# JerryX1110/Robust-Video-Object-Segmentation

Measured on AMD Instinct MI355X. Metric: frames/sec, AOC-Net matching + calibration hot path (480p, 3 objects), higher is better.
Workload: dtype f32; 1 GPU; cfg2: 121x213 stride-4 maps (480p), O=4 (3 objects + background), K=16 proxies, C=100, 60-frame clips, MEM_EVERY=5 (pool R=1..12), 20 Lloyd iterations, local windows 2..12, 10 IA gates + 4 conditioning blocks; sequences_per_gpu=2, proxy_mode=reference

## Files before the change

### robust-video-object-segmentation_amd/csrc/labels_kmeans.hip

```cpp
#include "aoc_common.h"
#include <stdlib.h>
#include <algorithm>
#include <string.h>

namespace {

constexpr int LP_BLOCK = 256;

__global__ __launch_bounds__(LP_BLOCK) void label_flags_kernel(const float *__restrict__ labels, int n, int n_obj,
                                                                uint32_t *__restrict__ right_bits,
                                                                uint32_t *__restrict__ wrong_bits,
                                                                int32_t *__restrict__ block_counts, int n_blocks) {
    __shared__ int32_t wave_cnt[LP_BLOCK / 64][AOC_MAX_OBJECTS + 1];
    const int row = blockIdx.x * LP_BLOCK + threadIdx.x;
    uint32_t right = 0, wrong = 0;
    if (row < n) {
        const float *l = labels + (size_t)row * n_obj;
        float sum = 0.0f;
        for (int o = 0; o < n_obj; ++o) {
            float v = l[o];
            sum += v;
            if (v > 0.9f) right |= 1u << o;
            if (v < 0.1f) wrong |= 1u << o;
        }
// ... 2058 lines not shown
        if constexpr (NF > 1) { if (!skip[1]) { st[1] = ks_chunk_exact<1, NF>(to_float(1), cur, blocks_here, lane, ks_big); to_int(1); } }
        if constexpr (NF > 2) {
            if (!skip[2]) { st[2] = ks_chunk_exact<2, NF>(to_float(2), cur, blocks_here, lane, ks_big); to_int(2); }
            if (!skip[3]) { st[3] = ks_chunk_exact<3, NF>(to_float(3), cur, blocks_here, lane, ks_big); to_int(3); }
        }
        ks_tex += KS_CLK() - ks_tb;
        if (ks_big) KS_STAT(2, 1);
#pragma unroll
        for (int f = 0; f < NF; ++f) note_crossing(f, c, e_in[f]);
    }
#pragma unroll
    for (int f = 0; f < NF; ++f) st[f] = to_float(f);
    if (ks_big) { KS_STAT(0, KS_CLK() - ks_t0); KS_STAT(1, ks_tsum); KS_STAT(4, ks_tex); }
    if (lane == 0) {
        const float fc = (float)cnt;
#pragma unroll
        for (int f = 0; f < NF; ++f) out[f] = st[f] / fc;
        if (pred.e0) {
#pragma unroll
            for (int f = 0; f < NF; ++f) {
                const size_t idx = ((size_t)s * kmax + j) * C + NF * q + f;
                pred.e0[idx] = (int8_t)pe0[f];
#pragma unroll
                for (int i = 0; i < KP_CROSS; ++i) {
                    pred.cidx[idx * KP_CROSS + i] = (uint16_t)pci[f][i];
                    pred.ce[idx * KP_CROSS + i] = (int8_t)pce[f][i];
                }
            }
        }
    }
}

constexpr int OS_BATCH = 128;
constexpr int OS_FP = 7;
constexpr int OS_LD = 32;
constexpr int OS_NPROD = 7;
constexpr int OS_PP = OS_BATCH * OS_FP / (OS_NPROD * 64);
constexpr int OS_DEPTH = 6;
static_assert(OS_PP * OS_NPROD * 64 == OS_BATCH * OS_FP && OS_DEPTH % 2 == 0 && OS_FP * 4 <= OS_LD, "ordered-sum geometry");
inline int os_groups(int C) { return (C / 4 + OS_FP - 1) / OS_FP; }
__device__ __forceinline__ int os_groups_dev(int C) { return (C / 4 + OS_FP - 1) / OS_FP; }

template <int MODE>
__device__ __forceinline__ void os_ordered_sum_body(int j, int s, int grp, float *__restrict__ os_lds, const float *__restrict__ pool, uint32_t pool_bytes, int C,
                                                    const int32_t *__restrict__ seg_off, const int32_t *__restrict__ seg_k,
                                                    const int32_t *__restrict__ counts, const int32_t *__restrict__ cbase,
                                                    const uint32_t *__restrict__ moff, int kmax, float *__restrict__ dst,
                                                    int member_cap, float *__restrict__ head_state) {
    if (j >= seg_k[s]) return;
    const int oc = s * kmax + j;
    const int cnt_all = counts[oc];
    const int f0 = grp * OS_FP * 4;
    const int nfeat = min(OS_FP * 4, C - f0);
    float *out = ((MODE == 0) ? dst + (size_t)oc * C : dst + (((size_t)s * 2 + 1) * kmax + j) * C) + f0;
    if (cnt_all == 0) {
        if (MODE == 1 && (int)threadIdx.x < nfeat) out[threadIdx.x] = 0.0f;
        return;
    }
    const bool head_only = member_cap > 0 && cnt_all > member_cap;
    const int cnt = head_only ? member_cap : cnt_all;
    const int wave = threadIdx.x >> 6, lane = aoc_lane();
    const int nb = (cnt + OS_BATCH - 1) / OS_BATCH;

    if (wave == 0) {
        const bool active = lane < nfeat;
        const float *col = os_lds + (active ? lane : 0);
        float sum = 0.0f;
        for (int b = 0; b < nb; ++b) {
            __syncthreads();
            const float *t = col + (b & 1) * OS_BATCH * OS_LD;
            float xa[16], xb[16];
#pragma unroll
            for (int u = 0; u < 16; ++u) xa[u] = t[u * OS_LD];
#pragma unroll
            for (int g = 0; g < OS_BATCH / 16; g += 2) {
#pragma unroll
                for (int u = 0; u < 16; ++u) xb[u] = t[((g + 1) * 16 + u) * OS_LD];
#pragma unroll
                for (int u = 0; u < 16; ++u) sum = sum + xa[u];
                if (g + 2 < OS_BATCH / 16) {
#pragma unroll
                    for (int u = 0; u < 16; ++u) xa[u] = t[((g + 2) * 16 + u) * OS_LD];
                }
#pragma unroll
                for (int u = 0; u < 16; ++u) sum = sum + xb[u];
            }
        }
        if (active) {
            if (head_only) head_state[(size_t)oc * C + f0 + lane] = sum;
            else out[lane] = sum / (float)cnt;
        }
        return;
    }

    const uint32_t *list = moff + seg_off[s] + cbase[oc];
    __amdgpu_buffer_rsrc_t rsrc = __builtin_amdgcn_make_buffer_rsrc(const_cast<float *>(pool), 0, pool_bytes, 0x00020000);
    const int p = (wave - 1) * 64 + lane;
    const int c4 = C >> 2;
    int prow[OS_PP];
    uint32_t pbyte[OS_PP];
    bool pvalid[OS_PP];
#pragma unroll
    for (int i = 0; i < OS_PP; ++i) {
        const int idx = i * (OS_NPROD * 64) + p;
        prow[i] = idx / OS_FP;
        const int piece = idx - prow[i] * OS_FP;
        pvalid[i] = grp * OS_FP + piece < c4;
        pbyte[i] = (uint32_t)(grp * OS_FP + piece) * 16u;
    }
    auto load_offs = [&](int b, uint32_t (&o)[OS_PP]) {
#pragma unroll
        for (int i = 0; i < OS_PP; ++i) {
            const int m = b * OS_BATCH + prow[i];
            const uint32_t v = list[min(m, cnt - 1)];
            o[i] = (b < nb && pvalid[i] && m < cnt) ? v + pbyte[i] : KU_INVALID_OFF;
        }
    };
    auto load_rows = [&](const uint32_t (&o)[OS_PP], u32x4 (&d)[OS_PP]) {
#pragma unroll
        for (int i = 0; i < OS_PP; ++i) d[i] = __builtin_amdgcn_raw_buffer_load_b128(rsrc, o[i], 0, 0);
    };
    auto write_rows = [&](int b, const u32x4 (&d)[OS_PP]) {
        float *base = os_lds + (b & 1) * OS_BATCH * OS_LD;
#pragma unroll
        for (int i = 0; i < OS_PP; ++i)
            *reinterpret_cast<u32x4 *>(base + prow[i] * OS_LD + ((pbyte[i] >> 2) - f0)) = d[i];
    };
    u32x4 d[OS_DEPTH][OS_PP];
    uint32_t o[2][OS_PP];
    {
        uint32_t po[OS_DEPTH + 2][OS_PP];
#pragma unroll
        for (int k = 0; k < OS_DEPTH + 2; ++k) load_offs(k, po[k]);
#pragma unroll
        for (int k = 0; k < OS_DEPTH; ++k) load_rows(po[k], d[k]);
        write_rows(0, d[0]);
        load_rows(po[OS_DEPTH], d[0]);
#pragma unroll
        for (int i = 0; i < OS_PP; ++i) o[1][i] = po[OS_DEPTH + 1][i];
    }
    for (int b0 = 0; b0 < nb; b0 += OS_DEPTH) {
#pragma unroll
        for (int k = 0; k < OS_DEPTH; ++k) {
            const int b = b0 + k;
            if (b < nb) {
                __syncthreads();
                if (b + 1 < nb) write_rows(b + 1, d[(k + 1) % OS_DEPTH]);
                load_offs(b + 2 + OS_DEPTH, o[k & 1]);
                load_rows(o[(k + 1) & 1], d[(k + 1) % OS_DEPTH]);
            }
        }
    }
}
#ifndef AOC_OD_NPROD
#define AOC_OD_NPROD 3
#endif
#ifndef AOC_OD_DEPTH
#define AOC_OD_DEPTH 1
#endif
constexpr int OD_NPROD = AOC_OD_NPROD;
constexpr int OD_HALF = 64;
constexpr int OD_BATCH = OD_NPROD * OD_HALF;
constexpr int OD_DEPTH = AOC_OD_DEPTH;
constexpr int OD_NB = OD_DEPTH + 1;
constexpr int OD_LD = OS_FP * 4;
constexpr int OD_BATCH_BYTES = OD_BATCH * OD_LD * 4;
constexpr int OD_RING_FLOATS = OD_NB * OD_BATCH * OD_LD;
constexpr int OD_OPS = OS_FP + 1;
constexpr int OD_LDS_FLOATS = OD_RING_FLOATS + OD_NB * OD_BATCH;
static_assert(OD_DEPTH * OD_OPS < 64 && OD_NPROD >= 1 && OD_NPROD <= 3, "vmcnt is a 6-bit counter; the launch has four waves");

__device__ __forceinline__ void od_glds4(const void *gsrc, uint32_t lds_dst) {
    unsigned keep;
    asm volatile("s_mov_b32 %0, m0\n\ts_mov_b32 m0, %2\n\ts_nop 0\n\tglobal_load_lds_dword %1, off\n\ts_mov_b32 m0, %0"
                 : "=&s"(keep) : "v"(gsrc), "s"(lds_dst) : "memory");
}
__device__ __forceinline__ void od_glds16(uint32_t byte_off, const void *base, uint32_t lds_dst) {
    unsigned keep;
    asm volatile("s_mov_b32 %0, m0\n\ts_mov_b32 m0, %3\n\ts_nop 0\n\tglobal_load_lds_dwordx4 %1, %2\n\ts_mov_b32 m0, %0"
                 : "=&s"(keep) : "v"(byte_off), "s"(base), "s"(lds_dst) : "memory");
}
template <int N>
__device__ __forceinline__ void od_wait_vm() { asm volatile("s_waitcnt vmcnt(%0)" ::"n"(N) : "memory"); }
__device__ __forceinline__ void od_barrier() {
    __builtin_amdgcn_s_waitcnt(0xc07f);
    __builtin_amdgcn_s_barrier();
    asm volatile("" ::: "memory");
}

template <int MODE>
__device__ __forceinline__ void os_head_dma_body(int j, int s, int grp, float *__restrict__ os_lds, const float *__restrict__ pool, int C,
                                                 const int32_t *__restrict__ seg_off, const int32_t *__restrict__ seg_k,
                                                 const int32_t *__restrict__ counts, const int32_t *__restrict__ cbase,
                                                 const uint32_t *__restrict__ moff, int kmax, float *__restrict__ dst, int member_cap,
                                                 float *__restrict__ head_state, KsPred pred) {
    const int wave = __builtin_amdgcn_readfirstlane(threadIdx.x >> 6), lane = aoc_lane();
    if (wave > OD_NPROD) return;
    if (j >= seg_k[s]) return;
    const int oc = s * kmax + j;
    const int cnt_all = counts[oc];
    const int f0 = grp * OS_FP * 4;
    const int nfeat = min(OS_FP * 4, C - f0);
    float *out = ((MODE == 0) ? dst + (size_t)oc * C : dst + (((size_t)s * 2 + 1) * kmax + j) * C) + f0;
    if (cnt_all == 0) {
        if (MODE == 1 && (int)threadIdx.x < nfeat) out[threadIdx.x] = 0.0f;
        return;
    }
    const bool head_only = member_cap > 0 && cnt_all > member_cap;
    const int cnt = head_only ? member_cap : cnt_all;
    const int nb = (cnt + OD_BATCH - 1) / OD_BATCH;
    auto wrap = [](int x) { return x >= OD_NB ? x - OD_NB : x; };

    if (wave == 0) {
        const bool active = lane < nfeat;
        const float *col = os_lds + (active ? lane : 0);
        float sum = 0.0f;
        int slot = 0;
        for (int b = 0; b < nb; ++b) {
            od_barrier();
            const float *t = col + slot * (OD_BATCH * OD_LD);
            constexpr int OD_G = 32, NG = OD_BATCH / OD_G;
            const int rem = (b + 1 < nb) ? OD_BATCH : cnt - b * OD_BATCH;
            float xa[OD_G], xb[OD_G];
#pragma unroll
            for (int u = 0; u < OD_G; ++u) xa[u] = t[u * OD_LD];
#pragma unroll
            for (int g = 0; g < NG; g += 2) {
                if (g + 1 < NG) {
#pragma unroll
                    for (int u = 0; u < OD_G; ++u) xb[u] = t[((g + 1) * OD_G + u) * OD_LD];
                }
                if (rem >= (g + 1) * OD_G) {
#pragma unroll
                    for (int u = 0; u < OD_G; ++u) sum = sum + xa[u];
                } else {
#pragma unroll
                    for (int u = 0; u < OD_G; ++u) sum = sum + (g * OD_G + u < rem ? xa[u] : 0.0f);
                }
                if (g + 2 < NG) {
#pragma unroll
                    for (int u = 0; u < OD_G; ++u) xa[u] = t[((g + 2) * OD_G + u) * OD_LD];
                }
                if (g + 1 < NG) {
                    if (rem >= (g + 2) * OD_G) {
#pragma unroll
                        for (int u = 0; u < OD_G; ++u) sum = sum + xb[u];
                    } else {
#pragma unroll
                        for (int u = 0; u < OD_G; ++u) sum = sum + ((g + 1) * OD_G + u < rem ? xb[u] : 0.0f);
                    }
                }
            }
            slot = wrap(slot + 1);
        }
        if (active) {
            if (head_only) head_state[(size_t)oc * C + f0 + lane] = sum;
            else out[lane] = sum / (float)cnt;
            if (!head_only && pred.e0) {
                const size_t idx = (size_t)oc * C + f0 + lane;
                const KsBinade bb = ks_binade(sum);
                pred.e0[idx] = (int8_t)(bb.ok ? (int)((__float_as_uint(sum) >> 23) & 0xff) - 127 : KC_UNSAFE);
                pred.cidx[idx * KP_CROSS] = (uint16_t)0xFFFF;
            }
        }
        return;
    }

    const int p = wave - 1;
    const uint32_t *list = moff + seg_off[s] + cbase[oc];
    const uint32_t lds_base = (uint32_t)reinterpret_cast<uintptr_t>(os_lds);
    const uint32_t offs_base = lds_base + OD_RING_FLOATS * 4 + (uint32_t)p * (OD_HALF * 4);
    const uint32_t *offs = reinterpret_cast<const uint32_t *>(os_lds + OD_RING_FLOATS) + p * OD_HALF;
    const int npiece = min(OS_FP, (C >> 2) - grp * OS_FP);
    int prow[OS_FP];
    uint32_t pbyte[OS_FP];
#pragma unroll
    for (int i = 0; i < OS_FP; ++i) {
        const int idx = i * 64 + lane;
        prow[i] = idx / OS_FP;
        const int piece = idx - prow[i] * OS_FP;
        pbyte[i] = (uint32_t)(grp * OS_FP + (piece < npiece ? piece : 0)) * 16u;
    }
    auto issue_offs = [&](int b, int slot) {
        od_glds4(list + min(b * OD_BATCH + p * OD_HALF + lane, cnt - 1), offs_base + (uint32_t)slot * (OD_BATCH * 4));
    };
    auto issue_rows = [&](int slot) {
        const uint32_t *o = offs + slot * OD_BATCH;
        uint32_t src[OS_FP];
#pragma unroll
        for (int i = 0; i < OS_FP; ++i) src[i] = o[prow[i]] + pbyte[i];
        const uint32_t d = lds_base + (uint32_t)slot * OD_BATCH_BYTES + (uint32_t)p * (OD_HALF * OD_LD * 4);
#pragma unroll
        for (int i = 0; i < OS_FP; ++i) od_glds16(src[i], pool, d + (uint32_t)i * 1024u);
    };
#pragma unroll
    for (int x = 0; x < OD_DEPTH; ++x) issue_offs(x, x);
    od_wait_vm<0>();
#pragma unroll
    for (int i = 0; i < OD_DEPTH; ++i) {
        issue_offs(OD_DEPTH + i, wrap(OD_DEPTH + i));
        issue_rows(i);
    }
    int slot = 0;
    for (int b = 0; b < nb; ++b) {
        od_wait_vm<(OD_DEPTH - 1) * OD_OPS>();
        od_barrier();
        const int slot_d = wrap(slot + OD_DEPTH);
        issue_offs(b + 2 * OD_DEPTH, wrap(slot_d + OD_DEPTH));
        issue_rows(slot_d);
        slot = wrap(slot + 1);
    }
    od_wait_vm<0>();
}
template <int MODE>
__global__ __launch_bounds__((OS_NPROD + 1) * 64) void km_ordered_sum_kernel(const float *__restrict__ pool, uint32_t pool_bytes, int C,
                                                                              const int32_t *__restrict__ seg_off, const int32_t *__restrict__ seg_k,
                                                                              const int32_t *__restrict__ counts, const int32_t *__restrict__ cbase,
                                                                              const uint32_t *__restrict__ moff, int kmax, float *__restrict__ dst,
                                                                              int member_cap, float *__restrict__ head_state) {
    __shared__ __attribute__((aligned(16))) float os_lds[2 * OS_BATCH * OS_LD];
    os_ordered_sum_body<MODE>(blockIdx.x, blockIdx.y, blockIdx.z, os_lds, pool, pool_bytes, C, seg_off, seg_k, counts, cbase, moff, kmax, dst, member_cap, head_state);
}
template <int MODE, bool DMA>
__global__ __launch_bounds__(DMA ? 256 : (OS_NPROD + 1) * 64) void km_heads_chunk_sums_kernel(const float *__restrict__ pool, uint32_t pool_bytes, int C,
                                                                                   const int32_t *__restrict__ seg_off, const int32_t *__restrict__ seg_k,
                                                                                   const int32_t *__restrict__ counts, const int32_t *__restrict__ cbase,
                                                                                   const uint32_t *__restrict__ moff, int kmax, int n_seg, float *__restrict__ dst,
                                                                                   int member_cap, float *__restrict__ head_state,
                                                                                   const int32_t *__restrict__ owner_cluster, const int32_t *__restrict__ owner_local,
                                                                                   float *__restrict__ csum, int start_chunk, int xcd_aware,
                                                                                   KsPred pred, int spec_fold, int8_t *__restrict__ cexp,
                                                                                   int32_t *__restrict__ cinc0, int32_t *__restrict__ cinc1,
                                                                                   const int32_t *__restrict__ cchunk, int n_chunks_grid, int n_fold_groups) {
    __shared__ __attribute__((aligned(16))) float os_lds[DMA ? (OD_LDS_FLOATS > 2 * OS_BATCH * OS_LD ? OD_LDS_FLOATS : 2 * OS_BATCH * OS_LD) : 2 * OS_BATCH * OS_LD];
    static_assert(sizeof(float) * 2 * OS_BATCH * OS_LD >= sizeof(uint32_t) * KS_CHUNK + sizeof(float4) * 256, "the chunk role's buffers fit the head role's");
    static_assert(2 * OS_BATCH * OS_LD >= KC_FOLD_LDS_FLOATS, "the fold role's buffers fit the head role's");
    const int n_head = kmax * n_seg * os_groups_dev(C);
    const int b = blockIdx.x;
    if (b < n_head) {
        const int n_cl = kmax * n_seg, groups = os_groups_dev(C);
        const int blk = b / (8 * groups), rem = b - blk * (8 * groups);
        const int pc = min(8, n_cl - blk * 8);
        int grp = rem / pc, c = blk * 8 + rem - grp * pc;
        if (!xcd_aware) { c = b % n_cl; grp = b / n_cl; }
        const int j = c % kmax, s = c / kmax;
        if (DMA) os_head_dma_body<MODE>(j, s, grp, os_lds, pool, C, seg_off, seg_k, counts, cbase, moff, kmax, dst, member_cap, head_state, pred);
        else os_ordered_sum_body<MODE>(j, s, grp, os_lds, pool, pool_bytes, C, seg_off, seg_k, counts, cbase, moff, kmax, dst, member_cap, head_state);
        return;
    }
    if (threadIdx.x >= 256) return;
    if (DMA && spec_fold) {
        static_assert(!DMA || OD_LDS_FLOATS >= KC_WIDE_LDS_FLOATS, "the wide fold's tile fits the heads' ring");
        kc_chunk_fold_wide_body(b - n_head, os_lds, pool, C, seg_off, counts, cbase, moff, kmax, owner_cluster, owner_local, cexp, cinc0, cinc1, start_chunk,
                                n_chunks_grid, n_fold_groups, xcd_aware, pred);
        return;
    }
    uint32_t *loffs = reinterpret_cast<uint32_t *>(os_lds);
    float4 *part = reinterpret_cast<float4 *>(os_lds + KS_CHUNK);
    kc_chunk_sum_body(b - n_head, loffs, part, pool, C, seg_off, counts, cbase, moff, kmax, owner_cluster, owner_local, csum, start_chunk);
}

__global__ __launch_bounds__(64) void km_proxy_finish_kernel(const float *__restrict__ centroids, const int32_t *__restrict__ seg_k,
                                                              const int32_t *__restrict__ counts, int kmax, int C,
                                                              float *__restrict__ proxies, float *__restrict__ proxy_sqnorm) {
    const int s = blockIdx.y, j = blockIdx.x, lane = threadIdx.x;
    const int k = seg_k[s];
    float *p0 = proxies + (((size_t)s * 2 + 0) * kmax + j) * C;
    float *p1 = proxies + (((size_t)s * 2 + 1) * kmax + j) * C;
    if (j >= k) {
        for (int t = lane; t < C; t += 64) { p0[t] = 0.0f; p1[t] = 0.0f; }
        if (lane == 0) {
            proxy_sqnorm[((size_t)s * 2 + 0) * kmax + j] = INFINITY;
            proxy_sqnorm[((size_t)s * 2 + 1) * kmax + j] = INFINITY;
        }
        return;
    }
    const float *c = centroids + ((size_t)s * kmax + j) * C;
    float n0 = 0.0f, n1 = 0.0f;
    for (int t = lane; t < C; t += 64) {
        const float cv = c[t];
        p0[t] = cv;
        n0 += cv * cv;
        const float av = p1[t];
        n1 += av * av;
    }
    n0 = aoc_wave_sum(n0);
    n1 = aoc_wave_sum(n1);
    if (lane == 0) {
        proxy_sqnorm[((size_t)s * 2 + 0) * kmax + j] = n0;
        proxy_sqnorm[((size_t)s * 2 + 1) * kmax + j] = (counts[s * kmax + j] > 0) ? n1 : INFINITY;
    }
}

struct KsWorkspace {
    float *rownorm;
    uint16_t *rank16;
    int32_t *hist, *counts, *cbase;
    uint32_t *moff;
    int nb_max;
    int nch_cap;
    int32_t *cchunk, *owner_cluster, *owner_local, *cinc0, *cinc1;
    float *csum, *head;
    int8_t *cexp;
    uint32_t *cflag;
    int seg_chunks_max;
    KsPred pred;
};
inline size_t ks_pred_bytes(int n_seg, int kmax) {
    const size_t n = (size_t)n_seg * kmax * (AOC_MAX_CHANNELS / 2);
    return aoc_align_up(n, 256) + aoc_align_up(n * KP_CROSS * 2, 256) + aoc_align_up(n * KP_CROSS, 256);
}
inline int ks_chunk_capacity(int64_t cap, int n_seg, int kmax) { return (int)(cap / KS_CHUNK) + n_seg * (kmax + 1) + 2; }
inline size_t ks_workspace_bytes(int64_t cap, int n_seg, int kmax) {
    const size_t nb = (size_t)(cap + 255) / 256 + 1;
    const size_t nch = (size_t)ks_chunk_capacity(cap, n_seg, kmax);
    return aoc_align_up((size_t)cap * 4, 256) + aoc_align_up((size_t)cap * 2, 256) + aoc_align_up((size_t)n_seg * nb * kmax * 4, 256) +
           3 * aoc_align_up((size_t)n_seg * kmax * 4, 256) + aoc_align_up(((size_t)cap + 64) * 4, 256) + 2 * aoc_align_up(nch * 4, 256) +
           3 * aoc_align_up(nch * AOC_MAX_CHANNELS / 2 * 4, 256) + aoc_align_up(nch * AOC_MAX_CHANNELS / 2, 256) +
           aoc_align_up((size_t)n_seg * kmax * (AOC_MAX_CHANNELS / 2) * 4, 256) + aoc_align_up(nch * 8 * 4, 256) + ks_pred_bytes(n_seg, kmax);
}
inline KsWorkspace ks_carve(void *workspace, int64_t cap, int n_seg, int kmax, int64_t seg_bound = 0) {
    KsWorkspace w;
    char *p = static_cast<char *>(workspace);
    const size_t nb = (size_t)(cap + 255) / 256 + 1;
    w.nb_max = (int)((seg_bound > 0 && seg_bound < cap) ? (size_t)(seg_bound + 255) / 256 + 1 : nb);
    w.seg_chunks_max = (int)(((seg_bound > 0 && seg_bound < cap) ? seg_bound : cap) / KS_CHUNK + 1);
    w.rownorm = reinterpret_cast<float *>(p); p += aoc_align_up((size_t)cap * 4, 256);
    w.rank16 = reinterpret_cast<uint16_t *>(p); p += aoc_align_up((size_t)cap * 2, 256);
    w.hist = reinterpret_cast<int32_t *>(p); p += aoc_align_up((size_t)n_seg * nb * kmax * 4, 256);
    w.counts = reinterpret_cast<int32_t *>(p); p += aoc_align_up((size_t)n_seg * kmax * 4, 256);
    w.cbase = reinterpret_cast<int32_t *>(p); p += aoc_align_up((size_t)n_seg * kmax * 4, 256);
    w.cchunk = reinterpret_cast<int32_t *>(p); p += aoc_align_up((size_t)n_seg * kmax * 4, 256);
    w.moff = reinterpret_cast<uint32_t *>(p); p += aoc_align_up(((size_t)cap + 64) * 4, 256);
    const size_t nch = (size_t)ks_chunk_capacity(cap, n_seg, kmax);
    w.nch_cap = (int)nch;
    w.owner_cluster = reinterpret_cast<int32_t *>(p); p += aoc_align_up(nch * 4, 256);
    w.owner_local = reinterpret_cast<int32_t *>(p); p += aoc_align_up(nch * 4, 256);
    w.csum = reinterpret_cast<float *>(p); p += aoc_align_up(nch * AOC_MAX_CHANNELS / 2 * 4, 256);
    w.cinc0 = reinterpret_cast<int32_t *>(p); p += aoc_align_up(nch * AOC_MAX_CHANNELS / 2 * 4, 256);
    w.cinc1 = reinterpret_cast<int32_t *>(p); p += aoc_align_up(nch * AOC_MAX_CHANNELS / 2 * 4, 256);
    w.cexp = reinterpret_cast<int8_t *>(p); p += aoc_align_up(nch * AOC_MAX_CHANNELS / 2, 256);
    w.head = reinterpret_cast<float *>(p); p += aoc_align_up((size_t)n_seg * kmax * (AOC_MAX_CHANNELS / 2) * 4, 256);
    w.cflag = reinterpret_cast<uint32_t *>(p); p += aoc_align_up(nch * 8 * 4, 256);
    {
        const size_t n = (size_t)n_seg * kmax * (AOC_MAX_CHANNELS / 2);
        w.pred.e0 = reinterpret_cast<int8_t *>(p); p += aoc_align_up(n, 256);
        w.pred.cidx = reinterpret_cast<uint16_t *>(p); p += aoc_align_up(n * KP_CROSS * 2, 256);
        w.pred.ce = reinterpret_cast<int8_t *>(p);
    }
    return w;
}

inline int km_xcd_aware() {
    static const int on = AOC_DEV_ENV_INT("AOC_KM_XCD", 1) != 0;
    return on;
}
static const int KS_HEAD_CHUNKS = AOC_DEV_ENV_INT("AOC_KM_HEAD_CHUNKS", 20) > 0 ? AOC_DEV_ENV_INT("AOC_KM_HEAD_CHUNKS", 20) : 20;
constexpr int KC_INLINE_PREDICT_CHUNKS = 800;
inline int ks_sum_mode() {
    static const int mode = [] {
        const char *e = AOC_DEV_ENV("AOC_KM_SUM");
        if (e && strcmp(e, "scan") == 0) return 0;
        if (e && strcmp(e, "ordered") == 0) return 1;
        return 2;
    }();
// ... 195 lines not shown

    hipLaunchKernelGGL(km_init_kernel, dim3(kmax, n_seg), dim3(64), 0, st, pool, C, rows, seg_offsets, seg_k, init_rows, kmax,
                       centroids, cnorm, cluster_counts);
    const dim3 agrid((unsigned)((seg_bound + 255) / 256), (unsigned)n_seg);
    const dim3 sgrid((unsigned)((seg_bound + 256 * KSS_BLOCKS - 1) / (256 * KSS_BLOCKS)), (unsigned)n_seg);
    const size_t lds = ((size_t)kmax * C + kmax) * sizeof(float);
    const size_t lds_fast = lds + (size_t)4 * kmax * sizeof(int32_t);
    const int nf = (C + 63) / 64;
    const bool use_mfma = fast && mfma_assign && C == 100 && kmax <= 64;
    if (use_mfma) {
        const size_t per_r = ((size_t)((kmax + 15) / 16) * 16 * 116 + ((kmax + 15) / 16) * 16) * sizeof(float) + 256;
        const size_t fixed_r = (size_t)4 * 16 * 116 * sizeof(float) + (size_t)4 * kmax * sizeof(int32_t);
        const bool rep_path = n_rep > 1 && (km_rep_lds_budget((kmax + 15) / 16) - fixed_r) / per_r >= 2 && AOC_DEV_ENV_INT("AOC_KM_ASSIGN_REP", 1) != 0;
        const int lim = rep_path ? n_seg / n_rep : n_seg;
        const int64_t bound = rep_path ? std::min<int64_t>(rows_capacity / n_rep + 1, rows_capacity) : rows_capacity;
        hipLaunchKernelGGL(km_rownorm_kernel, dim3((unsigned)((bound + 255) / 256)), dim3(256), 0, st, pool, C, rows, seg_offsets, lim, rownorm);
    }
    for (int it = 0; it < iters; ++it) {
        const int first = (it == 0);
        if (use_mfma) {
            const int kt = (kmax + 15) / 16;
            const int64_t gcap = kt == 1 ? (int64_t)km_assign_grid_cap() * 3 / 2 : km_assign_grid_cap();
            bool rep_done = false;
            {
                const size_t fixed = (size_t)4 * 16 * 116 * sizeof(float) + (size_t)4 * kmax * sizeof(int32_t);
                const size_t per = ((size_t)kt * 16 * 116 + kt * 16) * sizeof(float) + 256;
                const int fit = (int)std::min<size_t>(16, (km_rep_lds_budget(kt) - fixed) / per);
                static const bool rep_off = AOC_DEV_ENV_INT("AOC_KM_ASSIGN_REP", 1) == 0;
                if (n_rep > 1 && fit >= 2 && !rep_off) {
                    const int n_groups = (n_rep + fit - 1) / fit;
                    const int n_grp = (n_rep + n_groups - 1) / n_groups;
                    const int n_base = n_seg / n_rep;
                    const size_t rlds = fixed + (size_t)n_grp * per;
                    const int64_t base_rows = std::min<int64_t>(rows_capacity / n_rep, seg_bound * n_base);
                    const unsigned rgrid = (unsigned)std::min<int64_t>((base_rows / 256 + n_base) * n_groups, gcap);
#define AOC_KAR(KT)                                                                                                                                        \
    do {                                                                                                                                                   \
        static const bool ok = hipFuncSetAttribute(reinterpret_cast<const void *>(km_assign_mfma_rep_kernel<25, KT>),                                     \
                                                   hipFuncAttributeMaxDynamicSharedMemorySize, (int)km_rep_lds_budget(KT) + 2048) == hipSuccess;           \
        if (!ok) return AOC_ERR_LAUNCH;                                                                                                                    \
        hipLaunchKernelGGL((km_assign_mfma_rep_kernel<25, KT>), dim3(rgrid), dim3(256), rlds, st, pool, C, rows, seg_offsets, seg_k, n_base, n_rep, n_grp, \
                           centroids, kmax, labels, ws.rank16, ws.hist, ws.nb_max, rownorm);                                                               \
    } while (0)
                    if (kt == 1) AOC_KAR(1); else if (kt == 2) AOC_KAR(2); else if (kt == 3) AOC_KAR(3); else AOC_KAR(4);
#undef AOC_KAR
                    rep_done = true;
                }
            }
            if (!rep_done) {
            const size_t alds = ((size_t)kt * 16 * 116 + kt * 16 + (size_t)4 * 16 * 116) * sizeof(float) + (size_t)4 * kmax * sizeof(int32_t);
            const unsigned pgrid = (unsigned)std::min<int64_t>(std::min<int64_t>(rows_capacity, seg_bound * n_seg) / 256 + n_seg, gcap);
#define AOC_KA(KT) hipLaunchKernelGGL((km_assign_mfma_kernel<25, KT>), dim3(pgrid), dim3(256), alds, st, pool, C, rows, seg_offsets, seg_k, n_seg, centroids, \
                                      kmax, labels, ws.rank16, ws.hist, ws.nb_max, rownorm)
            if (kt == 1) AOC_KA(1); else if (kt == 2) AOC_KA(2); else if (kt == 3) AOC_KA(3); else AOC_KA(4);
#undef AOC_KA
            }
        } else if (fast) {
            if (C <= 100)
                hipLaunchKernelGGL(km_assign_rank_kernel<25>, agrid, dim3(256), lds_fast, st, pool, C, rows, seg_offsets, seg_k, centroids, kmax, labels,
                                   ws.rank16, ws.hist, ws.nb_max, rownorm, first);
            else
                hipLaunchKernelGGL(km_assign_rank_kernel<32>, agrid, dim3(256), lds_fast, st, pool, C, rows, seg_offsets, seg_k, centroids, kmax, labels,
                                   ws.rank16, ws.hist, ws.nb_max, rownorm, first);
        }
        if (fast) {
            hipLaunchKernelGGL(km_scan_scatter_kernel, sgrid, dim3(256), 0, st, rows, (const int32_t *)nullptr, seg_offsets, seg_k, n_seg, labels, ws.rank16,
                               ws.hist, ws.nb_max, kmax, (uint32_t)C * 4u, ws.moff, cluster_counts, ws.cbase, ws.cchunk, ws.owner_cluster, ws.owner_local,
                               ws.nch_cap, ws.cflag);
            ks_launch_sums<0>(st, pool, pool_bytes, C, seg_offsets, seg_k, cluster_counts, ws, kmax, n_seg, centroids, it > 0);
            continue;
        }
        if ((C % 4) == 0 && C <= 100)
            hipLaunchKernelGGL(km_assign_kernel<25>, agrid, dim3(256), lds, st, pool, C, rows, seg_offsets, seg_k, centroids, cnorm, kmax, labels, rownorm, first);
        else if ((C % 4) == 0 && C <= 128)
            hipLaunchKernelGGL(km_assign_kernel<32>, agrid, dim3(256), lds, st, pool, C, rows, seg_offsets, seg_k, centroids, cnorm, kmax, labels, rownorm, first);
        else
            hipLaunchKernelGGL(km_assign_generic_kernel, agrid, dim3(256), 0, st, pool, C, rows, seg_offsets, seg_k, centroids, cnorm, kmax, labels, rownorm, first);
        const dim3 ugrid(kmax, n_seg);
#define AOC_KU(NF) hipLaunchKernelGGL((km_accumulate_kernel<NF, 0>), ugrid, dim3(64), 0, st, pool, C, rows, seg_offsets, seg_k, labels, kmax, centroids, cnorm, cluster_counts, (float *)nullptr, (float *)nullptr)
        if (nf == 1) AOC_KU(1); else if (nf == 2) AOC_KU(2); else if (nf == 3) AOC_KU(3); else AOC_KU(4);
#undef AOC_KU
    }
    AOC_RETURN_IF_LAUNCH_FAILED();
    return AOC_OK;
}

int aoc_kmeans_replicate(const int32_t *rows, const int32_t *seg_offsets, const int32_t *seg_k, int n_seg, int n_rep, int64_t rows_capacity,
                         int32_t *rows_out, int32_t *seg_offsets_out, int32_t *seg_k_out, aoc_stream_t stream) {
    if (!rows || !seg_offsets || !seg_k || !rows_out || !seg_offsets_out || !seg_k_out) return AOC_ERR_INVALID_ARG;
    if (n_seg < 1 || n_rep < 1 || rows_capacity < 1 || (int64_t)n_rep * rows_capacity >= (1ll << 31)) return AOC_ERR_INVALID_ARG;
    const int64_t span = rows_capacity > n_seg + 1 ? rows_capacity : n_seg + 1;
    hipLaunchKernelGGL(km_replicate_kernel, dim3((unsigned)((span + 255) / 256), (unsigned)n_rep), dim3(256), 0, aoc_hip_stream(stream), rows, seg_offsets,
                       seg_k, n_seg, n_rep, rows_capacity, rows_out, seg_offsets_out, seg_k_out);
    AOC_RETURN_IF_LAUNCH_FAILED();
    return AOC_OK;
}

int aoc_kmeans_replicate_levels(const int32_t *rows, const int32_t *seg_offsets, int n_seg, int n_rep, const int32_t *levels_host, int n_levels,
                                int64_t rows_capacity, int32_t *rows_out, int32_t *seg_offsets_out, int32_t *seg_k_out, aoc_stream_t stream) {
    if (!rows || !seg_offsets || !levels_host || !rows_out || !seg_offsets_out || !seg_k_out) return AOC_ERR_INVALID_ARG;
    if (n_seg < 1 || n_rep < 1 || n_levels < 1 || rows_capacity < 1 || (int64_t)n_rep * rows_capacity >= (1ll << 31)) return AOC_ERR_INVALID_ARG;
    if (n_levels > 8) return AOC_ERR_UNSUPPORTED;
    if (rows_out == rows && n_rep != 1) return AOC_ERR_INVALID_ARG;
    KmLevels kl;
    kl.n = n_levels;
    for (int i = 0; i < 8; ++i) {
        kl.k[i] = i < n_levels ? levels_host[i] : 0;
        if (i < n_levels && (levels_host[i] < 0 || levels_host[i] > AOC_MAX_CLUSTERS)) return AOC_ERR_INVALID_ARG;
    }
    const int64_t span = rows_capacity > n_seg + 1 ? rows_capacity : n_seg + 1;
    hipLaunchKernelGGL(km_replicate_levels_kernel, dim3((unsigned)((span + 255) / 256), (unsigned)n_rep), dim3(256), 0, aoc_hip_stream(stream), rows,
                       seg_offsets, n_seg, n_rep, kl, rows_capacity, rows_out, seg_offsets_out, seg_k_out);
    AOC_RETURN_IF_LAUNCH_FAILED();
    return AOC_OK;
}

size_t aoc_build_proxies_workspace_bytes(int64_t rows_capacity, int n_seg, int kmax) {
    if (rows_capacity < 0 || n_seg < 1 || kmax < 1) return 0;
    return ks_workspace_bytes(rows_capacity, n_seg, kmax);
}

int aoc_build_proxies(const float *pool, int64_t pool_rows, int C, const int32_t *fg_rows, const int32_t *seg_offsets, const int32_t *seg_k,
                      const int32_t *labels, const float *centroids, int n_seg, int kmax, int64_t rows_capacity,
                      float *proxies, float *proxy_sqnorm, void *workspace, size_t workspace_bytes, aoc_stream_t stream) {
    if (!pool || !fg_rows || !seg_offsets || !seg_k || !labels || !centroids || !proxies || !proxy_sqnorm) return AOC_ERR_INVALID_ARG;
    if (C < 1 || n_seg < 1 || kmax < 1) return AOC_ERR_INVALID_ARG;
    if (C > AOC_MAX_CHANNELS || kmax > AOC_MAX_CLUSTERS || n_seg > 65535) return AOC_ERR_UNSUPPORTED;
    hipStream_t st = aoc_hip_stream(stream);
    const dim3 grid(kmax, n_seg);
    const int nf = (C + 63) / 64;
    const bool fast = (C % 4) == 0 && C <= 128 && pool_rows > 0 && rows_capacity > 0 && (uint64_t)pool_rows * C * 4 < 0xFFFFFF00ull && workspace &&
                      workspace_bytes >= aoc_build_proxies_workspace_bytes(rows_capacity, n_seg, kmax);
    if (fast) {
        const int64_t seg_bound = (pool_rows < rows_capacity) ? pool_rows : rows_capacity;
        KsWorkspace ws = ks_carve(workspace, rows_capacity, n_seg, kmax, seg_bound);
        const dim3 agrid((unsigned)((seg_bound + 255) / 256), (unsigned)n_seg);
        hipLaunchKernelGGL(km_rank_only_kernel, agrid, dim3(256), 0, st, seg_offsets, seg_k, labels, kmax, ws.rank16, ws.hist, ws.nb_max);
        const dim3 sgrid((unsigned)((seg_bound + 256 * KSS_BLOCKS - 1) / (256 * KSS_BLOCKS)), (unsigned)n_seg);
        hipLaunchKernelGGL(km_scan_scatter_kernel, sgrid, dim3(256), 0, st, (const int32_t *)nullptr, fg_rows, seg_offsets, seg_k, n_seg, labels, ws.rank16,
                           ws.hist, ws.nb_max, kmax, (uint32_t)C * 4u, ws.moff, ws.counts, ws.cbase, ws.cchunk, ws.owner_cluster, ws.owner_local,
                           ws.nch_cap, ws.cflag);
        ks_launch_sums<1>(st, pool, (uint32_t)((uint64_t)pool_rows * C * 4), C, seg_offsets, seg_k, ws.counts, ws, kmax, n_seg, proxies);
        hipLaunchKernelGGL(km_proxy_finish_kernel, grid, dim3(64), 0, st, centroids, seg_k, ws.counts, kmax, C, proxies, proxy_sqnorm);
        AOC_RETURN_IF_LAUNCH_FAILED();
        return AOC_OK;
    }
#define AOC_KP(NF) hipLaunchKernelGGL((km_accumulate_kernel<NF, 1>), grid, dim3(64), 0, st, pool, C, fg_rows, seg_offsets, seg_k, labels, kmax, const_cast<float *>(centroids), (float *)nullptr, (int32_t *)nullptr, proxies, proxy_sqnorm)
    if (nf == 1) AOC_KP(1); else if (nf == 2) AOC_KP(2); else if (nf == 3) AOC_KP(3); else AOC_KP(4);
#undef AOC_KP
    AOC_RETURN_IF_LAUNCH_FAILED();
    return AOC_OK;
}

#ifdef AOC_KS_STATS
int aoc_debug_ks_stats(unsigned long long *out8_host, int reset) {
    if (hipMemcpyFromSymbol(out8_host, HIP_SYMBOL(aoc_ks_stats), 8 * sizeof(unsigned long long)) != hipSuccess) return AOC_ERR_LAUNCH;
    if (reset) {
        unsigned long long z[8] = {0, 0, 0, 0, 0, 0, 0, 0};
        if (hipMemcpyToSymbol(HIP_SYMBOL(aoc_ks_stats), z, sizeof(z)) != hipSuccess) return AOC_ERR_LAUNCH;
    }
    return AOC_OK;
}
#endif

}
```

Before: 444.2 frames/s.

## Restructure ordered-sum DMA ring into per-producer 64-row slots with staggered issue

Replaces the batched ring, where three producer waves jointly filled a 192-row batch, with a six-slot ring of 64-row slots. Each producer owns two slots and advances round-robin. Producers split row transfers into a first and a rest portion across successive barriers, and the consumer sums one 64-row slot per barrier, prefetching the next slot's first half. The aim is finer-grained overlap between global-to-LDS loads and the reduction while keeping the LDS footprint at three workgroups per CU. Optional cycle-counter profiling is added behind a compile flag. The change brings more barriers per row and more complex waitcnt bookkeeping.

```diff
diff --git a/robust-video-object-segmentation_amd/csrc/labels_kmeans.hip b/robust-video-object-segmentation_amd/csrc/labels_kmeans.hip
--- a/robust-video-object-segmentation_amd/csrc/labels_kmeans.hip
+++ b/robust-video-object-segmentation_amd/csrc/labels_kmeans.hip
@@ -2234,23 +2234,32 @@
         }
     }
 }
-#ifndef AOC_OD_NPROD
-#define AOC_OD_NPROD 3
+#ifndef AOC_OD_FIRST
+#define AOC_OD_FIRST 4
 #endif
-#ifndef AOC_OD_DEPTH
-#define AOC_OD_DEPTH 1
+constexpr int OD_NPROD = 3;
+constexpr int OD_SLOT = 64;
+constexpr int OD_OWN = 2;
+constexpr int OD_NSLOT = OD_NPROD * OD_OWN;
+constexpr int OD_LD = OS_FP * 4;
+constexpr int OD_SLOT_BYTES = OD_SLOT * OD_LD * 4;
+constexpr int OD_RING_FLOATS = OD_NSLOT * OD_SLOT * OD_LD;
+constexpr int OD_OPS = OS_FP + 1;
+constexpr int OD_FIRST = AOC_OD_FIRST;
+constexpr int OD_LDS_FLOATS = OD_RING_FLOATS + OD_NSLOT * OD_SLOT;
+static_assert(OD_OWN * OD_OPS < 64, "vmcnt is a 6-bit counter");
+static_assert(OD_SLOT * OD_LD * 4 == OS_FP * 64 * 16 && OD_FIRST >= 1 && OD_FIRST <= OS_FP, "seven 1 KiB transfers tile a slot");
+static_assert(OD_LDS_FLOATS * 4 <= 44544, "three workgroups per CU: not more LDS than the two-slot ring had");
+
+#ifdef AOC_OD_PROF
+__device__ unsigned long long aoc_od_prof[8];
+#define OD_CLK() ((long long)__builtin_readcyclecounter())
+#define OD_PROF_ADD(i, n) atomicAdd(&aoc_od_prof[i], (unsigned long long)(n))
+#else
+#define OD_CLK() 0ll
+#define OD_PROF_ADD(i, n) do { } while (0)
 #endif
-constexpr int OD_NPROD = AOC_OD_NPROD;
-constexpr int OD_HALF = 64;
-constexpr int OD_BATCH = OD_NPROD * OD_HALF;
-constexpr int OD_DEPTH = AOC_OD_DEPTH;
-constexpr int OD_NB = OD_DEPTH + 1;
-constexpr int OD_LD = OS_FP * 4;
-constexpr int OD_BATCH_BYTES = OD_BATCH * OD_LD * 4;
-constexpr int OD_RING_FLOATS = OD_NB * OD_BATCH * OD_LD;
-constexpr int OD_OPS = OS_FP + 1;
-constexpr int OD_LDS_FLOATS = OD_RING_FLOATS + OD_NB * OD_BATCH;
-static_assert(OD_DEPTH * OD_OPS < 64 && OD_NPROD >= 1 && OD_NPROD <= 3, "vmcnt is a 6-bit counter; the launch has four waves");
+constexpr int OD_PROF_MIN = 5000;
 
 __device__ __forceinline__ void od_glds4(const void *gsrc, uint32_t lds_dst) {
     unsigned keep;
@@ -2290,51 +2299,58 @@
     }
     const bool head_only = member_cap > 0 && cnt_all > member_cap;
     const int cnt = head_only ? member_cap : cnt_all;
-    const int nb = (cnt + OD_BATCH - 1) / OD_BATCH;
-    auto wrap = [](int x) { return x >= OD_NB ? x - OD_NB : x; };
+    const int ns = (cnt + OD_SLOT - 1) / OD_SLOT;
+    __builtin_amdgcn_s_waitcnt(0x0f70);
 
     if (wave == 0) {
         const bool active = lane < nfeat;
         const float *col = os_lds + (active ? lane : 0);
         float sum = 0.0f;
+        constexpr int OD_G = OD_SLOT / 2;
+        float xa[OD_G], xb[OD_G];
+        long long pc_bar = 0, pc_add = 0;
+        (void)pc_bar; (void)pc_add;
+        {
+            const long long c0 = OD_CLK();
+            od_barrier();
+            pc_bar += OD_CLK() - c0;
+        }
+        long long pc_t = OD_CLK();
+#pragma unroll
+        for (int u = 0; u < OD_G; ++u) xa[u] = col[u * OD_LD];
         int slot = 0;
-        for (int b = 0; b < nb; ++b) {
-            od_barrier();
-            const float *t = col + slot * (OD_BATCH * OD_LD);
-            constexpr int OD_G = 32, NG = OD_BATCH / OD_G;
-            const int rem = (b + 1 < nb) ? OD_BATCH : cnt - b * OD_BATCH;
-            float xa[OD_G], xb[OD_G];
-#pragma unroll
-            for (int u = 0; u < OD_G; ++u) xa[u] = t[u * OD_LD];
-#pragma unroll
-            for (int g = 0; g < NG; g += 2) {
-                if (g + 1 < NG) {
-#pragma unroll
-                    for (int u = 0; u < OD_G; ++u) xb[u] = t[((g + 1) * OD_G + u) * OD_LD];
-                }
-                if (rem >= (g + 1) * OD_G) {
-#pragma unroll
-                    for (int u = 0; u < OD_G; ++u) sum = sum + xa[u];
-                } else {
-#pragma unroll
-                    for (int u = 0; u < OD_G; ++u) sum = sum + (g * OD_G + u < rem ? xa[u] : 0.0f);
-                }
-                if (g + 2 < NG) {
-#pragma unroll
-                    for (int u = 0; u < OD_G; ++u) xa[u] = t[((g + 2) * OD_G + u) * OD_LD];
-                }
-                if (g + 1 < NG) {
-                    if (rem >= (g + 2) * OD_G) {
-#pragma unroll
-                        for (int u = 0; u < OD_G; ++u) sum = sum + xb[u];
-                    } else {
-#pragma unroll
-                        for (int u = 0; u < OD_G; ++u) sum = sum + ((g + 1) * OD_G + u < rem ? xb[u] : 0.0f);
-                    }
-                }
-            }
-            slot = wrap(slot + 1);
-        }
+        for (int st = 0; st < ns; ++st) {
+            const float *t = col + slot * (OD_SLOT * OD_LD);
+            const int rem = (st + 1 < ns) ? OD_SLOT : cnt - st * OD_SLOT;
+#pragma unroll
+            for (int u = 0; u < OD_G; ++u) xb[u] = t[(OD_G + u) * OD_LD];
+            if (rem >= OD_G) {
+#pragma unroll
+                for (int u = 0; u < OD_G; ++u) sum = sum + xa[u];
+            } else {
+#pragma unroll
+                for (int u = 0; u < OD_G; ++u) sum = sum + (u < rem ? xa[u] : 0.0f);
+            }
+            slot = (slot + 1 == OD_NSLOT) ? 0 : slot + 1;
+            if (st + 1 < ns) {
+                const long long c0 = OD_CLK();
+                od_barrier();
+                const long long c1 = OD_CLK();
+                pc_add += c0 - pc_t; pc_bar += c1 - c0; pc_t = c1;
+                const float *tn = col + slot * (OD_SLOT * OD_LD);
+#pragma unroll
+                for (int u = 0; u < OD_G; ++u) xa[u] = tn[u * OD_LD];
+            }
+            if (rem >= 2 * OD_G) {
+#pragma unroll
+                for (int u = 0; u < OD_G; ++u) sum = sum + xb[u];
+            } else {
+#pragma unroll
+                for (int u = 0; u < OD_G; ++u) sum = sum + (OD_G + u < rem ? xb[u] : 0.0f);
+            }
+        }
+        pc_add += OD_CLK() - pc_t;
+        if (lane == 0 && cnt >= OD_PROF_MIN) { OD_PROF_ADD(0, cnt); OD_PROF_ADD(1, pc_bar); OD_PROF_ADD(2, pc_add); OD_PROF_ADD(7, 1); }
         if (active) {
             if (head_only) head_state[(size_t)oc * C + f0 + lane] = sum;
             else out[lane] = sum / (float)cnt;
@@ -2351,8 +2367,8 @@
     const int p = wave - 1;
     const uint32_t *list = moff + seg_off[s] + cbase[oc];
     const uint32_t lds_base = (uint32_t)reinterpret_cast<uintptr_t>(os_lds);
-    const uint32_t offs_base = lds_base + OD_RING_FLOATS * 4 + (uint32_t)p * (OD_HALF * 4);
-    const uint32_t *offs = reinterpret_cast<const uint32_t *>(os_lds + OD_RING_FLOATS) + p * OD_HALF;
+    const uint32_t offs_base = lds_base + OD_RING_FLOATS * 4;
+    const uint32_t *offs = reinterpret_cast<const uint32_t *>(os_lds + OD_RING_FLOATS);
     const int npiece = min(OS_FP, (C >> 2) - grp * OS_FP);
     int prow[OS_FP];
     uint32_t pbyte[OS_FP];
@@ -2363,36 +2379,75 @@
         const int piece = idx - prow[i] * OS_FP;
         pbyte[i] = (uint32_t)(grp * OS_FP + (piece < npiece ? piece : 0)) * 16u;
     }
-    auto issue_offs = [&](int b, int slot) {
-        od_glds4(list + min(b * OD_BATCH + p * OD_HALF + lane, cnt - 1), offs_base + (uint32_t)slot * (OD_BATCH * 4));
+    uint32_t src[OS_FP];
+    auto issue_offs = [&](int step, int slot) {
+        od_glds4(list + min(step * OD_SLOT + lane, cnt - 1), offs_base + (uint32_t)slot * (OD_SLOT * 4));
     };
-    auto issue_rows = [&](int slot) {
-        const uint32_t *o = offs + slot * OD_BATCH;
-        uint32_t src[OS_FP];
+    auto take_offs = [&](int slot) {
+        const uint32_t *o = offs + slot * OD_SLOT;
 #pragma unroll
         for (int i = 0; i < OS_FP; ++i) src[i] = o[prow[i]] + pbyte[i];
-        const uint32_t d = lds_base + (uint32_t)slot * OD_BATCH_BYTES + (uint32_t)p * (OD_HALF * OD_LD * 4);
-#pragma unroll
-        for (int i = 0; i < OS_FP; ++i) od_glds16(src[i], pool, d + (uint32_t)i * 1024u);
+        asm volatile("s_waitcnt lgkmcnt(0)" : "+v"(src[0]), "+v"(src[1]), "+v"(src[2]), "+v"(src[3]), "+v"(src[4]), "+v"(src[5]), "+v"(src[6]) : : "memory");
     };
-#pragma unroll
-    for (int x = 0; x < OD_DEPTH; ++x) issue_offs(x, x);
+    static_assert(OS_FP == 7, "take_offs names seven registers");
+    auto rows_first = [&](int slot) {
+        const uint32_t d = lds_base + (uint32_t)slot * OD_SLOT_BYTES;
+#pragma unroll
+        for (int i = 0; i < OD_FIRST; ++i) od_glds16(src[i], pool, d + (uint32_t)i * 1024u);
+    };
+    auto rows_rest = [&](int slot) {
+        const uint32_t d = lds_base + (uint32_t)slot * OD_SLOT_BYTES;
+#pragma unroll
+        for (int i = OD_FIRST; i < OS_FP; ++i) od_glds16(src[i], pool, d + (uint32_t)i * 1024u);
+    };
+    if (p < ns) issue_offs(p, p);
+    if (p + OD_NPROD < ns) issue_offs(p + OD_NPROD, p + OD_NPROD);
     od_wait_vm<0>();
 #pragma unroll
-    for (int i = 0; i < OD_DEPTH; ++i) {
-        issue_offs(OD_DEPTH + i, wrap(OD_DEPTH + i));
-        issue_rows(i);
-    }
-    int slot = 0;
-    for (int b = 0; b < nb; ++b) {
-        od_wait_vm<(OD_DEPTH - 1) * OD_OPS>();
+    for (int x = 0; x < OD_OWN; ++x) {
+        const int u = p + x * OD_NPROD;
+        if (u < ns) {
+            take_offs(u);
+            issue_offs(u + OD_NSLOT, u);
+            rows_first(u);
+            rows_rest(u);
+        }
+    }
+    for (int st = 0; st < p && st < ns; ++st) od_barrier();
+    long long pp_w = 0, pp_b = 0, pp_i = 0;
+    int n_own = 0;
+    (void)pp_w; (void)pp_b; (void)pp_i; (void)n_own;
+    int sl = p;
+    for (int u = p; u < ns; u += OD_NPROD) {
+        const long long t0 = OD_CLK();
+        if (u + OD_NPROD < ns) od_wait_vm<(OD_OWN - 1) * OD_OPS>();
+        else od_wait_vm<0>();
+        const long long t1 = OD_CLK();
         od_barrier();
-        const int slot_d = wrap(slot + OD_DEPTH);
-        issue_offs(b + 2 * OD_DEPTH, wrap(slot_d + OD_DEPTH));
-        issue_rows(slot_d);
-        slot = wrap(slot + 1);
+        long long t2 = OD_CLK(), t3 = t2, t4 = t2, t5 = t2;
+        if (u + 1 < ns) {
+            od_barrier();
+            t3 = OD_CLK();
+            const int nx = u + OD_NSLOT;
+            if (nx < ns) {
+                take_offs(sl);
+                issue_offs(nx + OD_NSLOT, sl);
+                rows_first(sl);
+            }
+            t5 = t4 = OD_CLK();
+            if (u + 2 < ns) {
+                od_barrier();
+                t5 = OD_CLK();
+                if (nx < ns) rows_rest(sl);
+            }
+        }
+        const long long t6 = OD_CLK();
+        pp_w += t1 - t0; pp_b += (t2 - t1) + (t3 - t2) + (t5 - t4); pp_i += (t4 - t3) + (t6 - t5);
+        ++n_own;
+        sl = (sl == p) ? p + OD_NPROD : p;
     }
     od_wait_vm<0>();
+    if (lane == 0 && cnt >= OD_PROF_MIN) { OD_PROF_ADD(3, n_own); OD_PROF_ADD(4, pp_w); OD_PROF_ADD(5, pp_b); OD_PROF_ADD(6, pp_i); }
 }
 template <int MODE>
 __global__ __launch_bounds__((OS_NPROD + 1) * 64) void km_ordered_sum_kernel(const float *__restrict__ pool, uint32_t pool_bytes, int C,
@@ -2894,6 +2949,16 @@
     return AOC_OK;
 }
 
+#ifdef AOC_OD_PROF
+int aoc_debug_od_prof(unsigned long long *out8_host, int reset) {
+    if (hipMemcpyFromSymbol(out8_host, HIP_SYMBOL(aoc_od_prof), 8 * sizeof(unsigned long long)) != hipSuccess) return AOC_ERR_LAUNCH;
+    if (reset) {
+        unsigned long long z[8] = {0, 0, 0, 0, 0, 0, 0, 0};
+        if (hipMemcpyToSymbol(HIP_SYMBOL(aoc_od_prof), z, sizeof(z)) != hipSuccess) return AOC_ERR_LAUNCH;
+    }
+    return AOC_OK;
+}
+#endif
 #ifdef AOC_KS_STATS
 int aoc_debug_ks_stats(unsigned long long *out8_host, int reset) {
     if (hipMemcpyFromSymbol(out8_host, HIP_SYMBOL(aoc_ks_stats), 8 * sizeof(unsigned long long)) != hipSuccess) return AOC_ERR_LAUNCH;
```

After: 441.2 frames/s. Within noise of the previous version (-0.7%).
